# orottier/web-audio-api-rs

Measured on AMD Instinct MI355X. Metric: render quanta/sec (48kHz, 128-frame), higher is better.
Workload: dtype f64

## Files before the change

web-audio-api-rs_amd/csrc/waa_internal.hpp:

```cpp
#pragma once
#include <cstdint>
#include <cstdlib>

#include "waa_conv_noise.hpp"

namespace waa {

inline const char* measure_switch(const char* name) {
#ifdef WAA_MEASURE
  return getenv(name);
#else
  (void)name;
  return nullptr;
#endif
}

void raise_lds_limit(const void* kernel);

constexpr int RQ = 128;
constexpr int TILE_K = 32;
constexpr int TILE = 64 * TILE_K;
constexpr int QUANTA_PER_TILE = TILE / RQ;
constexpr int MAX_OPS = 12;
constexpr int MAX_INPUTS = 4;
// ... 29 lines not shown
struct SrcSchedule {
  const QRec* qrec;
  const SlowRec* slow;
  const uint8_t* tile_fast;
};
struct SrcInst {
  const float* base;
  uint64_t ch_stride;
  uint64_t frames;
  uint32_t sched;
  uint32_t aligned;
  SrcSchedule sc;
  int64_t linear_start;
  uint32_t fast_prefix;
  uint32_t linear_all;
};

enum : int32_t { IN_SILENT = 0, IN_SIGNAL = 1, IN_SOURCE = 2, IN_CONSTANT = 3, IN_DELAYED = 4 };
struct InputRef {
  int32_t kind;
  int32_t nch;
  SignalRef sig;
  const SrcInst* src;
  const SrcSchedule* sched;
  ParamRef offset;
  const int64_t* active;
  double sample_rate;
  int32_t num_quanta;
  int32_t feedback;
  uint64_t valid;
  ParamRef gain;
  int32_t has_gain;
  uint32_t fast_tiles;
  float delay_lo, delay_hi;
};

enum : int32_t {
  OP_GAIN = 1,
  OP_BIQUAD = 2,
  OP_WAVESHAPER = 3,
  OP_STEREO_PAN = 4,
  OP_PANNER = 5,
  OP_MIX = 6,
  OP_IIR = 7,
  OP_PARAM_ADD = 8
};
struct OpDesc {
  int32_t kind;
  int32_t nch_in;
  int32_t nch_out;
  int32_t i1;
  int32_t i2;
  int32_t i0;
  ParamRef p0;
  ParamRef p1;
  ParamRef p2;
  ParamRef p3;
  ParamRef p4;
  const void* ptr0;
  void* ptr1;
  const void* ptr2;
  uint64_t u0;
};

struct ChainDesc {
  int32_t n_inputs;
  int32_t in_nch;
  int32_t in_interp;
  int32_t n_ops;
  InputRef in[MAX_INPUTS];
  OpDesc ops[MAX_OPS];
  SignalRef out;
  uint32_t n_inst;
  uint32_t n_tiles;
  uint32_t n_quanta;
  uint32_t xcd_remap;
  uint32_t tile0, tile1;
  int32_t lds_curve_op;
  int32_t tile_major;
  uint32_t persist_block;
  uint32_t pad;
};

struct BiquadStreamDesc {
  InputRef in;
  const double* coefs;
  uint64_t coef_stride;
  int32_t vary;
  int32_t pad0;
  double* state;
  const double* hp;
  ParamRef gain[2];
  int32_t n_gain;
  int32_t nch;
  SignalRef out;
  uint32_t n_inst;
  uint32_t n_tiles;
  uint32_t n_quanta;
  uint32_t dup_out;
  uint32_t tile0, tile1;
};
void launch_biquad_stream(const BiquadStreamDesc& d, void* stream);
constexpr int BIQUAD_SCAN_PW = 88;
struct BiquadScanCtl {
  uint32_t* counter;
  uint32_t counter_base[8];
  double* payload;
  const double* pw;
  uint32_t* error;
};
void launch_biquad_scan_powers(const double* coefs, uint64_t coef_stride, double* pw, uint32_t n_inst, void* stream);
void launch_biquad_scan(const BiquadStreamDesc& d, const BiquadScanCtl& ctl, uint32_t* issued, void* stream);

constexpr int BIQUAD_HT_WORDS = 2 * TILE + 8;
struct BiquadLanesDesc {
  InputRef in;
  const double* coefs;
  double* ht;
  double* z;
  double* sin;
  double* state;
  ParamRef gain[2];
  int32_t n_gain, nch;
  SignalRef out;
  uint32_t n_inst, n_tiles, n_quanta, tile0, tile1;
  uint32_t fast_tiles;
  uint32_t lt0, lt1;
  uint32_t debug, pad;
};
void launch_biquad_tile_digest(const BiquadLanesDesc& d, void* stream);
void launch_biquad_lanes(const BiquadLanesDesc& d, void* stream);

struct IirStreamDesc {
  InputRef in;
  const double* coef;
  const double* pow;
  double* state;
  int32_t ns;
  int32_t nch;
  SignalRef out;
  uint32_t n_inst;
  uint32_t n_tiles;
  uint32_t n_quanta;
  uint32_t exact;
  uint32_t tile0, tile1;
  uint32_t coef_stride, pow_stride;
};
int iir_padded_states(int n_states);
void launch_iir_stream(const IirStreamDesc& d, void* stream);

struct CompRow {
  float thr, lo, hi, half_knee;
  float knee_partial, ratio, makeup, pad;
  float a_tau, a_one, r_tau, r_one;
};
struct CompDesc {
  SignalRef in;
  uint64_t in_valid;
  SignalRef out;
  float* xl;
  const CompRow* rows;
  uint32_t row_inst_stride, row_q_stride;
  uint32_t n_inst, n_quanta;
  uint64_t frames;
  uint32_t delay_frames;
  int32_t nch;
};
void launch_compressor_level(const CompDesc& d, void* stream);
void launch_compressor_detector(const CompDesc& d, void* stream);
void launch_compressor_apply(const CompDesc& d, void* stream);

enum : int32_t { RT_CHANNEL = 0, RT_DOWN2 = 1, RT_DOWN4 = 2, RT_DOWN6 = 3 };
struct RouteTerm {
  const float* base;
  uint64_t inst_stride, ch_stride;
  int32_t mode;
  int32_t ch;
};
struct RouteDesc {
  SignalRef out;
  const RouteTerm* terms;
  const uint32_t* row_off;
  uint32_t n_inst, rows;
  uint64_t frames;
};
void launch_route(const RouteDesc& d, void* stream);

struct ConvTerm {
  int32_t in_ch, ir_ch, out_ch, pad;
};
struct Cplx {
  float re, im;
};
struct ConvDesc {
  SignalRef in, out;
  int32_t n_terms;
  int32_t cin, cout;
  int32_t n;
  int32_t block;
  int32_t parts;
  int32_t nb;
  int32_t fft3;
  ConvTerm terms[4];
  const Cplx* H;
  Cplx* X;
  Cplx* Y;
  const Cplx* tw;
  const float* ir;
  uint64_t ir_len;
  uint64_t frames;
  uint64_t in_valid;
  uint32_t n_inst, n_pairs;
  int32_t ir_nch, pad1;
  int32_t kb0, kb1;
  int32_t mac_grid_order, pad2;
  const double* pre_coefs;
  uint64_t pre_coef_stride;
  double* pre_state;
  uint64_t ir_inst_stride;
  int32_t per_inst, pad3;
};
struct AnalyserDesc {
  SignalRef sig;
  uint32_t n_inst;
  int32_t fft_size;
  uint64_t frames_written;
  float smoothing;
  float min_db, max_db;
  int32_t pad;
  const float* window;
  const Cplx* tw;
  const Cplx* tw_full;
  const float* prev;
  float* db_out;
  uint8_t* byte_out;
  float* time_out;
  const uint8_t* code;
  uint64_t code_stride;
};
void launch_analyser(const AnalyserDesc& d, void* stream);
struct AnalyserSeriesDesc {
  AnalyserDesc a;
  int32_t first, hop;
  int32_t pulls;
  int32_t run;
  int32_t stage_span;
  int32_t lin;
  uint64_t frames;
  float* db_out;
  uint8_t* byte_out;
  float* time_out;
  uint8_t* tbyte_out;
};
void analyser_series_shape(AnalyserSeriesDesc* d);
void launch_analyser_series_fft(const AnalyserSeriesDesc& d, void* stream);
void launch_analyser_series_smooth(const AnalyserSeriesDesc& d, void* stream);
void launch_analyser_series_bytes(const AnalyserSeriesDesc& d, void* stream);
void launch_analyser_series_time(const AnalyserSeriesDesc& d, void* stream);
constexpr int DIRECT_MAX_TAPS = 128;
void launch_conv_direct(const ConvDesc& d, void* stream);
void launch_conv_ir_spectra(const ConvDesc& d, void* stream);
void launch_conv_forward(const ConvDesc& d, void* stream);
void launch_conv_mac(const ConvDesc& d, void* stream);
void launch_conv_inverse(const ConvDesc& d, void* stream);
void launch_conv3_ir_spectra(const ConvDesc& d, void* stream);
void launch_conv3_forward(const ConvDesc& d, void* stream);
void launch_conv3_inverse(const ConvDesc& d, void* stream);
void launch_conv_inst_direct(const ConvDesc& d, void* stream);
void launch_conv_inst_mac(const ConvDesc& d, void* stream);

struct DelayDesc {
  SignalRef in, out;
  ParamRef delay;
  double sample_rate;
  uint64_t frames;
  int32_t num_quanta;
  int32_t nch;
  uint32_t n_inst;
  uint32_t n_quanta;
  uint32_t tile0, tile1;
  int32_t in_cycle;
  int32_t pad;
  double quantum_duration;
};
void launch_delay(const DelayDesc& d, void* stream);


struct OscDesc {
  ParamRef frequency, detune;
  const double* start;
  const double* stop;
  const float* table;
  int32_t table_len;
  int32_t type;
  SignalRef out;
  uint64_t frames;
  uint32_t n_inst;
  uint32_t n_quanta;
  double sample_rate;
  const struct OscQuantum* table_q;
  const uint32_t* tq_row;
  const int64_t* active;
  const double* start_ratio;
  double* seg_phase;
  ParamRef post_gain[2];
  int32_t n_post;
  int32_t post_dup;
  const struct OscQuantum* fm_q;
  const uint32_t* fm_row;
  const float* fm_table;
  int32_t fm_table_len, fm_type;
  ParamRef fm_gain;
  int32_t fm_has_gain;
  float fm_min, fm_max, fm_default;
  int32_t pa_on;
  float pa_min, pa_max, pa_default;
  ParamRef pa_intrinsic;
};
constexpr int OSC_SEGMENTS = 8;
struct OscQuantum {
  double phase;
  double incr;
  int16_t first, end;
  int32_t outside_nyquist;
};
void launch_osc(const OscDesc& d, void* stream);

enum : int32_t { LI_NODE = 0, LI_DELAY_W = 1, LI_DELAY_R = 2 };
constexpr int LOOP_MAX_ITEMS = 24;
struct LoopItem {
  int32_t kind;
  int32_t nch_in;
  int32_t nch_out;
  int32_t interp;
  int32_t n_in;
  int32_t in_item[MAX_INPUTS];
  int32_t in_nch[MAX_INPUTS];
  SignalRef in_sig[MAX_INPUTS];
  SignalRef out;
  OpDesc op;
  int32_t writer_item;
  int32_t in_cycle;
  int32_t num_quanta;
  int32_t pad;
};
struct LoopDesc {
  const LoopItem* items;
  int32_t n_items;
  uint32_t n_inst;
  uint32_t n_quanta;
  uint32_t no_scan;
  double sample_rate;
  double quantum_duration;
};
void launch_loop(const LoopDesc& d, void* stream);

constexpr int DYN_MAX_IN = 8;
constexpr int DYN_MAX_ITEMS = 48;
constexpr int DYN_STATE = 20;
constexpr uint32_t CODE_SILENT = 0x80u;
enum : int32_t { DI_NODE = 0, DI_DELAY_W = 1, DI_DELAY_R = 2 };
enum : int32_t {
  DK_PASS = 0,
  DK_GAIN = 1, DK_BIQUAD = 2, DK_IIR = 3, DK_WAVESHAPER = 4, DK_STEREO_PAN = 5, DK_PANNER = 6,
  DK_CONV_IN = 7
};
struct DynInput {
  int32_t item;
  int32_t nch;
  SignalRef sig;
  const uint8_t* code;
  const uint32_t* remap;
  uint64_t code_stride;
};
struct DynItem {
  int32_t kind;
  int32_t dk;
  int32_t cc, mode, interp;
  int32_t n_in;
  int32_t nch_pub;
  int32_t publish_upmix;
  int32_t compact_ch1;
  int32_t flags;
  int32_t writer_item;
  int32_t in_cycle;
  int32_t num_quanta;
  int32_t pad;
  DynInput in[DYN_MAX_IN];
  OpDesc op;
  ParamRef alt1, alt2;
  SignalRef out;
  uint8_t* out_code;
  uint32_t* aux32;
  uint64_t code_stride;
  SignalRef xline;
  const uint32_t* xaux32;
  int32_t* xstate;
  int32_t pmod_n;
  int32_t pmod_item[4];
  float pmod_min, pmod_max, pmod_def;
};
struct DynDesc {
  const DynItem* items;
  int32_t n_items;
  uint32_t n_inst;
  uint32_t n_quanta;
  uint32_t no_scan;
  int32_t cmax;
  int32_t n_stages;
  int32_t stage_begin[9];
  int32_t pad;
  double sample_rate;
  double quantum_duration;
  unsigned long long* cycles;
  uint32_t q0, q1;
  double* save_f;
  int32_t* save_i;
  uint32_t split_ok, q_split;
};
void launch_dyn(const DynDesc& d, void* stream);
inline int dyn_planes(int cmax) { return cmax > 16 ? 32 : cmax > 8 ? 16 : cmax > 6 ? 8 : cmax > 2 ? 6 : 2; }
constexpr int DYN_MAX_STAGES = 8;
size_t dyn_lds_bytes(int n_items, int cmax, int stages = 1);
struct ConvCodeDesc {
  const uint8_t* in_code;
  uint8_t* out_code;
  uint64_t code_stride;
  uint64_t impulse_length;
  int32_t ir_nch;
  uint32_t n_inst, n_quanta;
  int32_t cout;
  uint8_t* clean;
  SignalRef out;
  uint32_t q0, q1;
  int32_t* state;
  int32_t noise, in_test_nch;
  SignalRef in;
  ConvNoiseIr nir[4];
};
constexpr int CONV_CODE_STATE_INTS = 4 + 4 * 4;
void launch_conv_codes(const ConvCodeDesc& d, void* stream);

struct BiquadCoefDesc {
  ParamRef frequency, detune, q, gain;
  double* coefs;
  uint64_t n_frames;
  uint64_t frames_padded;
  uint32_t rows;
  int32_t type;
  float sample_rate;
  int32_t lane_major;
};
void launch_biquad_coefs(const BiquadCoefDesc& d, void* stream);
constexpr int HP_WORDS = 72;
struct BiquadHpDesc {
  const double* coefs;
  double* hp;
  uint32_t n_tiles;
  uint32_t pad;
};
void launch_biquad_hp(const BiquadHpDesc& d, void* stream);

struct PannerGeomDesc {
  ParamRef p[15];
  const uint8_t* single;
  uint64_t single_stride;
  const uint8_t* dev_len[9];
  float *az, *gl_mono, *gr_mono, *gl_stereo, *gr_stereo, *dg, *cg;
  uint64_t n_frames;
  uint32_t rows;
  int32_t distance_model;
  double ref_distance, max_distance, rolloff;
  float cone_inner, cone_outer, cone_outer_gain;
  int32_t pad;
};
void launch_panner_geom(const PannerGeomDesc& d, void* stream);

struct TlEvent {
  int32_t type;
  float value;
  double time;
  double time_constant;
  double cancel_time;
  double duration;
  int32_t cancelled;
  int32_t curve_off;
  int32_t curve_len;
  int32_t pad;
};
struct TlHeader {
  float minv, maxv, defv, intrinsic;
  int32_t a_rate;
  int32_t ev_off;
  int32_t n_events;
  int32_t pad;
};
struct TimelineDesc {
  const TlHeader* hdr;
  const TlEvent* events;
  TlEvent* work;
  const float* curves;
  float* out;
  uint8_t* lens;
  uint64_t out_stride;
  uint32_t rows;
  uint32_t n_quanta;
  double sample_rate;
};
void launch_timeline(const TimelineDesc& d, void* stream);

constexpr int32_t LINK_SKIP = -2, LINK_FRESH = -1;
struct LinkDesc {
  const uint8_t* in_code;
  uint8_t* out_code;
  int32_t* prev;
  uint64_t code_stride, prev_stride;
  uint32_t n_inst, n_quanta;
  int32_t kind;
  int32_t can_propagate_silence;
  uint32_t tail_frames;
  int32_t pad;
  uint32_t q0, q1;
  int32_t* state;
};
void launch_link(const LinkDesc& d, void* stream);

struct QGemmDesc {
  const float* A;
  const uint16_t* A16;
  int32_t M, Kh;
  const float* src;
  uint64_t src_inst, src_ch, src_q;
  float* dst;
  uint64_t dst_inst, dst_ch, dst_q;
  const int32_t* prev;
  uint64_t prev_stride;
  const float* curve;
  int32_t curve_n;
  int32_t nch;
  uint32_t n_inst, n_quanta;
};
void launch_qgemm(const QGemmDesc& d, void* stream);

struct OsFftDesc {
  const float* src;
  uint64_t src_inst, src_ch;
  float* dst;
  uint64_t dst_inst, dst_ch;
  const int32_t* prev;
  uint64_t prev_stride;
  const float* curve;
  int32_t curve_n;
  int32_t R;
  const float* tables;
  const float* tw256;
  float* trash;
  int32_t nch;
  uint32_t n_inst, n_quanta;
  uint32_t seg_len, n_seg;
  uint32_t q0, q1;
};
void launch_osfft(const OsFftDesc& d, void* stream);
size_t osfft_lds_bytes(int R, int curve_n);

struct HrtfQ {
  int32_t v[3];
  float w[3];
  float gain;
  int32_t pad;
};
constexpr int HRTF_MAX_TAPS = 1280;
struct HrtfDesc {
  SignalRef in, out;
  const uint8_t* in_code;
  uint64_t code_stride;
  const int32_t* prev;
  uint64_t prev_stride;
  const float* hrir;
  const float* hstatic;
  const HrtfQ* table;
  uint32_t rows, per_row;
  int32_t taps;
  uint32_t n_inst, n_quanta;
  uint32_t q0, q1;
  int32_t pad;
  const float* fft_tables;
  const float* tw256;
  float* trash;
  uint32_t seg_len, n_seg;
  uint32_t n_seg_pad, pad2;
  const int32_t* jmax;
};
void launch_hrtf(const HrtfDesc& d, void* stream);
void launch_hrtf_fft(const HrtfDesc& d, void* stream);
void launch_hrtf_fft_tables(const float* pairs, uint32_t pair_stride, int taps, uint32_t rows, const double* cs_sn, float* out, void* stream);

struct DecodeDesc {
  const int16_t* pcm;
  float* out;
  uint64_t frames;
  uint64_t target_frames;
  uint64_t out_item_stride, out_ch_stride;
  uint32_t nch, n_items;
  int32_t resample;
  float scale;
};
void launch_pcm16_resample(const DecodeDesc& d, void* stream);
struct EncodeDesc {
  const float* in;
  int16_t* pcm;
  uint64_t frames, in_item_stride, in_ch_stride;
  uint32_t nch_in, nch_out, n_items, pad;
};
void launch_pcm16_pack(const EncodeDesc& d, void* stream);

void launch_chain(const ChainDesc& d, int cmax, void* stream);
struct EchoTail {
  int32_t n_inputs, in_nch, in_interp, store_line;
  int32_t ring_frames, sub_frames;
  InputRef in[MAX_INPUTS];
  int32_t alias[MAX_INPUTS];
  SignalRef out;
// ... 96 lines not shown
```

web-audio-api-rs_amd/csrc/waa_osc.hip:

```cpp
#include <hip/hip_runtime.h>

#include "waa_internal.hpp"

namespace waa {

namespace {
__device__ __forceinline__ double unroll_phase(double phase) {
  if (phase >= 1.) return phase - 1.;
  if (phase < 0.) return phase + 1.;
  return phase;
}
__device__ __forceinline__ double unroll_phase_unbounded(double phase) {
  const double r = fmod(phase, 1.);
  return r < 0. ? r + 1. : r;
}
__device__ __forceinline__ double poly_blep(double t, double dt) {
  if (t < dt) {
    t /= dt;
    return t + t - t * t - 1.0;
  } else if (t > 1.0 - dt) {
    t = (t - 1.0) / dt;
    return __builtin_fma(t, t, t) + t + 1.0;
  }
  return 0.0;
}
__device__ __forceinline__ float table_sample(const float* table, int len, double phase) {
  const double position = phase * (double)len;
  const double floored = floor(position);
  const int prev_index = (int)floored >= len ? 0 : (int)floored;
  int next_index = prev_index + 1;
  if (next_index == len) next_index = 0;
  const float k = (float)(position - floored);
  return __builtin_fmaf(table[prev_index], 1.f - k, table[next_index] * k);
}
__device__ __forceinline__ float waveform_sample(int type, const float* table, int table_len, double phase, double phase_incr) {
  switch (type) {
    case 1: {
      double sample = phase < 0.5 ? 1.0 : -1.0;
      sample += poly_blep(phase, phase_incr);
      sample -= poly_blep(unroll_phase(phase + 0.5), phase_incr);
      return (float)sample;
    }
    case 2: {
      const double ph = unroll_phase(phase + 0.5);
      double sample = 2.0 * ph - 1.0;
      sample -= poly_blep(ph, phase_incr);
      return (float)sample;
    }
    case 3: {
      double sample = -4. * phase + 2.;
      if (sample > 1.)
        sample = 2. - sample;
      else if (sample < -1.)
        sample = -2. - sample;
      return (float)sample;
    }
    default: return table_sample(table, table_len, phase);
  }
}
__device__ __forceinline__ float waveform_sample(const OscDesc& d, double phase, double phase_incr) {
  return waveform_sample(d.type, d.table, d.table_len, phase, phase_incr);
}
}

namespace {
__device__ __forceinline__ void osc_store(const OscDesc& d, uint32_t inst, float* out, uint64_t f0, float (&r)[4]) {
#pragma unroll
  for (int k = 0; k < 2; k++)
    if (k < d.n_post) {
      const float g = d.post_gain[k].base[inst];
      const bool mute = fabsf(g) <= 1e-6f, pass = fabsf(1.f - g) <= 1e-6f;
#pragma unroll
      for (int e = 0; e < 4; e++) r[e] = mute ? 0.f : (pass ? r[e] : r[e] * g);
    }
  if (d.pa_on) {
    const uint32_t q = (uint32_t)(f0 / RQ), qc = q < d.n_quanta ? q : d.n_quanta - 1;
    const float iv = d.pa_intrinsic.mode == 0 ? d.pa_intrinsic.base[inst] : d.pa_intrinsic.base[(uint64_t)inst * d.pa_intrinsic.stride + qc];
#pragma unroll
    for (int e = 0; e < 4; e++) {
      const float o1 = r[e] + iv;
      r[e] = o1 != o1 ? d.pa_default : fminf(fmaxf(o1, d.pa_min), d.pa_max);
    }
  }
  *reinterpret_cast<float4*>(out + f0) = make_float4(r[0], r[1], r[2], r[3]);
  if (d.post_dup) *reinterpret_cast<float4*>(out + d.out.ch_stride + f0) = make_float4(r[0], r[1], r[2], r[3]);
}
}

__global__ __launch_bounds__(64) void osc_kernel(const OscDesc d) {
  const uint32_t inst = blockIdx.x * 64 + threadIdx.x;
  if (inst >= d.n_inst) return;
  __builtin_amdgcn_s_setreg(1 | (6 << 6) | (1 << 11), 0);
  float* out = d.out.base + (uint64_t)inst * d.out.inst_stride;
  double start_time = d.start[inst];
  const double stop_time = d.stop[inst];
  const double sample_rate = d.sample_rate, dt = 1. / sample_rate, nyquist = sample_rate / 2.;
  double phase = 0.;
  bool started = false;
  const bool per_frame = d.frequency.mode == 2 || d.detune.mode == 2;
  for (uint32_t q = 0; q < d.n_quanta; q++) {
    const uint64_t f0 = (uint64_t)q * RQ;
    const double block_time = (double)f0 / sample_rate;
    const double next_block_time = block_time + dt * (double)RQ;
    float4* o4 = reinterpret_cast<float4*>(out + f0);
    if (stop_time <= block_time || start_time >= next_block_time) {
      for (int j = 0; j < RQ / 4; j++) o4[j] = make_float4(0.f, 0.f, 0.f, 0.f);
      continue;
    }
    double current_time = block_time;
    if (!started && start_time < current_time) start_time = current_time;
    auto generate = [&](bool outside_nyquist, double phase_incr) __attribute__((always_inline)) -> float {
      float v = 0.f;
      if (!(current_time < start_time || current_time >= stop_time)) {
        if (!started) {
          if (current_time > start_time) {
            const double ratio = (current_time - start_time) / dt;
            phase = outside_nyquist ? unroll_phase_unbounded(phase_incr * ratio) : unroll_phase(phase_incr * ratio);
          }
          started = true;
        }
        v = outside_nyquist ? 0.f : waveform_sample(d, phase, phase_incr);
        phase = outside_nyquist ? unroll_phase_unbounded(phase + phase_incr) : unroll_phase(phase + phase_incr);
      }
      current_time += dt;
      return v;
    };
    if (!per_frame) {
      const float freq = d.frequency.mode == 0 ? d.frequency.base[inst] : d.frequency.base[(uint64_t)inst * d.frequency.stride + q];
      const float detune = d.detune.mode == 0 ? d.detune.base[inst] : d.detune.base[(uint64_t)inst * d.detune.stride + q];
      const double computed_freq = (double)freq * exp2((double)detune / 1200.);
      const double phase_incr = computed_freq / sample_rate;
      const bool outside_nyquist = fabs(computed_freq) >= nyquist;
      const bool fully_active = started && start_time <= block_time && stop_time >= next_block_time;
      if (fully_active && !outside_nyquist) {
        for (int j = 0; j < RQ / 4; j++) {
          float r[4];
#pragma unroll
          for (int e = 0; e < 4; e++) {
            r[e] = waveform_sample(d, phase, phase_incr);
            phase = unroll_phase(phase + phase_incr);
          }
          o4[j] = make_float4(r[0], r[1], r[2], r[3]);
        }
      } else {
        for (int j = 0; j < RQ / 4; j++) {
          float r[4];
#pragma unroll
          for (int e = 0; e < 4; e++) r[e] = generate(outside_nyquist, phase_incr);
          o4[j] = make_float4(r[0], r[1], r[2], r[3]);
        }
      }
    } else {
      for (int j = 0; j < RQ / 4; j++) {
        float r[4];
#pragma unroll
        for (int e = 0; e < 4; e++) {
          const uint64_t f = f0 + j * 4 + e;
          const float freq = d.frequency.mode == 0   ? d.frequency.base[inst]
                             : d.frequency.mode == 1 ? d.frequency.base[(uint64_t)inst * d.frequency.stride + q]
                                                     : d.frequency.base[(uint64_t)inst * d.frequency.stride + f];
          const float detune = d.detune.mode == 0   ? d.detune.base[inst]
                               : d.detune.mode == 1 ? d.detune.base[(uint64_t)inst * d.detune.stride + q]
                                                    : d.detune.base[(uint64_t)inst * d.detune.stride + f];
          const double computed_freq = (double)freq * exp2((double)detune / 1200.);
          const double phase_incr = computed_freq / sample_rate;
          r[e] = generate(fabs(computed_freq) >= nyquist, phase_incr);
        }
        o4[j] = make_float4(r[0], r[1], r[2], r[3]);
      }
    }
  }
  for (uint64_t f = (uint64_t)d.n_quanta * RQ; f < d.frames; f += 4) *reinterpret_cast<float4*>(out + f) = make_float4(0.f, 0.f, 0.f, 0.f);
}

__global__ __launch_bounds__(256) void osc_par_kernel(const OscDesc d) {
  const uint32_t inst = blockIdx.y;
  const uint64_t f0 = ((uint64_t)blockIdx.x * 256 + threadIdx.x) * 4;
  if (f0 >= d.frames) return;
  __builtin_amdgcn_s_setreg(1 | (6 << 6) | (1 << 11), 0);
  float* out = d.out.base + (uint64_t)inst * d.out.inst_stride;
  const uint32_t q = (uint32_t)(f0 / RQ);
  float r[4] = {0.f, 0.f, 0.f, 0.f};
  if (q < d.n_quanta) {
    const OscQuantum oq = d.table_q[(uint64_t)d.tq_row[inst] * d.n_quanta + q];
    const int i0 = (int)(f0 % RQ);
#pragma unroll
    for (int e = 0; e < 4; e++) {
      const int i = i0 + e;
      if (i >= oq.first && i < oq.end && !oq.outside_nyquist) {
        const double x = __builtin_fma((double)(i - oq.first), oq.incr, oq.phase);
        double ph = x - floor(x);
        if (ph >= 1.) ph -= 1.;
        r[e] = waveform_sample(d, ph, oq.incr);
      }
    }
  }
  osc_store(d, inst, out, f0, r);
}

template <int PASS>
__global__ __launch_bounds__(64) void osc_scan_kernel(const OscDesc d) {
  const uint32_t inst = blockIdx.x;
  const uint32_t seg = blockIdx.y;
  const int lane = threadIdx.x;
  __builtin_amdgcn_s_setreg(1 | (6 << 6) | (1 << 11), 0);
  float* out = d.out.base + (uint64_t)inst * d.out.inst_stride;
  const int64_t first = d.active[(uint64_t)inst * 2], end = d.active[(uint64_t)inst * 2 + 1];
  const double ratio = d.start_ratio[inst];
  const double sample_rate = d.sample_rate, nyquist = sample_rate / 2.;
  const uint64_t groups = (d.frames + 255) / 256, per_seg = (groups + OSC_SEGMENTS - 1) / OSC_SEGMENTS;
  const uint64_t g_begin = (uint64_t)seg * per_seg * 256, g_end = g_begin + per_seg * 256 < d.frames ? g_begin + per_seg * 256 : d.frames;
  double carry = 0.;
  if (PASS == 1) {
    for (uint32_t sgm = 0; sgm < seg; sgm++) {
      carry += d.seg_phase[(uint64_t)inst * OSC_SEGMENTS + sgm];
      carry -= floor(carry);
    }
  }
  const bool det_const = d.detune.mode == 0;
  const double det_mul = det_const ? exp2((double)d.detune.base[inst] / 1200.) : 1.;
  for (uint64_t g0 = g_begin; g0 < g_end; g0 += 256) {
    const uint64_t f0 = g0 + (uint64_t)lane * 4;
    double incr[4];
    bool outside[4];
    OscQuantum mq4{};
    if (d.fm_q) {
      const uint64_t fq = f0 < (uint64_t)d.n_quanta * RQ ? f0 : (uint64_t)d.n_quanta * RQ - 1;
      mq4 = d.fm_q[(uint64_t)d.fm_row[inst] * d.n_quanta + fq / RQ];
    }
#pragma unroll
    for (int e = 0; e < 4; e++) {
      const uint64_t f = f0 + e;
      const uint64_t fc = f < (uint64_t)d.n_quanta * RQ ? f : (uint64_t)d.n_quanta * RQ - 1;
      const uint32_t q = (uint32_t)(fc / RQ);
      float freq = d.frequency.mode == 0   ? d.frequency.base[inst]
                   : d.frequency.mode == 1 ? d.frequency.base[(uint64_t)inst * d.frequency.stride + q]
                                           : d.frequency.base[(uint64_t)inst * d.frequency.stride + fc];
      if (d.fm_q) {
        const OscQuantum& mq = mq4;
        const int i = (int)(fc % RQ);
        float m = 0.f;
        if (i >= mq.first && i < mq.end && !mq.outside_nyquist) {
          const double x = __builtin_fma((double)(i - mq.first), mq.incr, mq.phase);
          double ph = x - floor(x);
          if (ph >= 1.) ph -= 1.;
          m = waveform_sample(d.fm_type, d.fm_table, d.fm_table_len, ph, mq.incr);
        }
        if (d.fm_has_gain) {
          const float g = d.fm_gain.mode == 0 ? d.fm_gain.base[inst] : d.fm_gain.base[(uint64_t)inst * d.fm_gain.stride + q];
          m = fabsf(g) <= 1e-6f ? 0.f : (fabsf(1.f - g) <= 1e-6f ? m : m * g);
        }
        float o1 = m + freq;
        freq = o1 != o1 ? d.fm_default : fminf(fmaxf(o1, d.fm_min), d.fm_max);
      }
      double computed_freq;
      if (det_const) {
        computed_freq = (double)freq * det_mul;
      } else {
        const float detune = d.detune.mode == 1 ? d.detune.base[(uint64_t)inst * d.detune.stride + q]
                                                : d.detune.base[(uint64_t)inst * d.detune.stride + fc];
        computed_freq = (double)freq * exp2((double)detune / 1200.);
      }
      incr[e] = computed_freq / sample_rate;
      outside[e] = fabs(computed_freq) >= nyquist;
    }
    double adv[4];
#pragma unroll
    for (int e = 0; e < 4; e++) {
      const int64_t f = (int64_t)(f0 + e);
      adv[e] = (f >= first && f < end) ? incr[e] : 0.;
      if (f == first) adv[e] += incr[e] * ratio;
    }
    const double local = ((adv[0] + adv[1]) + adv[2]) + adv[3];
    double incl = local;
#pragma unroll
    for (int sft = 1; sft < 64; sft <<= 1) {
      const double t = __shfl_up(incl, sft, 64);
      if (lane >= sft) incl += t;
    }
    if (PASS == 1) {
      double ph = carry + (incl - local);
      float r[4];
#pragma unroll
      for (int e = 0; e < 4; e++) {
        const int64_t f = (int64_t)(f0 + e);
        double p = ph;
        if (f == first) p += incr[e] * ratio;
        p -= floor(p);
        if (p >= 1.) p -= 1.;
        r[e] = (f >= first && f < end && !outside[e]) ? waveform_sample(d, p, incr[e]) : 0.f;
        ph += adv[e];
      }
      osc_store(d, inst, out, f0, r);
    }
    double total = __shfl(incl, 63, 64) + carry;
    total -= floor(total);
    carry = total;
  }
  if (PASS == 0 && lane == 0) d.seg_phase[(uint64_t)inst * OSC_SEGMENTS + seg] = carry;
}

void launch_osc(const OscDesc& d, void* stream) {
  if (d.table_q) {
    hipLaunchKernelGGL(osc_par_kernel, dim3((unsigned)((d.frames + 1023) / 1024), d.n_inst), dim3(256), 0, (hipStream_t)stream, d);
    return;
  }
  if (d.active) {
    hipLaunchKernelGGL(osc_scan_kernel<0>, dim3(d.n_inst, OSC_SEGMENTS), dim3(64), 0, (hipStream_t)stream, d);
    hipLaunchKernelGGL(osc_scan_kernel<1>, dim3(d.n_inst, OSC_SEGMENTS), dim3(64), 0, (hipStream_t)stream, d);
    return;
  }
  hipLaunchKernelGGL(osc_kernel, dim3((d.n_inst + 63) / 64), dim3(64), 0, (hipStream_t)stream, d);
}

}
```

web-audio-api-rs_amd/csrc/waa_plan_sources.cpp:

```cpp
#include <array>
#include <set>

#include "waa_host.hpp"
#include "waa_plan_parts.hpp"

namespace waa {
namespace host {

int widen_narrow_buffers(waa_batch* b, Node& n, uint32_t nch) {
  std::map<const float*, DeviceBuffer> done;
  for (auto& bf : n.bufs) {
    if (!bf.valid || bf.nch >= nch) continue;
    auto it = done.find(bf.base);
    if (it == done.end()) {
      const uint64_t stride = std::max<uint64_t>(bf.ch_stride, 4);
      float* d = nullptr;
      int e = dev_alloc(b, &d, (size_t)nch * stride, true);
      if (e) return e;
      const size_t all = (size_t)nch * stride * sizeof(float), plane = (size_t)bf.frames * sizeof(float);
      if (b->dry) {
        std::memset(d, 0, all);
        for (uint32_t c = 0; c < bf.nch && plane; c++) std::memcpy(d + (size_t)c * stride, bf.base + (size_t)c * bf.ch_stride, plane);
      } else {
        HIP_TRY(hipMemsetAsync(d, 0, all, b->stream));
// ... 130 lines not shown
      linear_all.push_back(all ? 1u : 0u);
      plan_note(b, "source node %u schedule %zu: tiles [0, %u) are one linear run from buffer frame %lld%s", id, scheds.size(), prefix,
                (long long)start0, all && prefix < b->n_tiles ? " (and so is the rest of the render)" : "");
    }
    SrcSchedule ds{};
    QRec* dq = nullptr;
    int e = dev_upload(b, &dq, so.qrec);
    if (e) return e;
    ds.qrec = dq;
    if (so.any_slow) {
      SlowRec* dsr = nullptr;
      e = dev_upload(b, &dsr, so.slow);
      if (e) return e;
      ds.slow = dsr;
    }
    uint8_t* dtf = nullptr;
    e = dev_upload(b, &dtf, so.tile_fast);
    if (e) return e;
    ds.tile_fast = dtf;
    si.sched = (uint32_t)scheds.size();
    scheds.push_back(ds);
    if (!automated) {
      dedup[key] = si.sched;
      last_key = key;
      last_sched = si.sched;
      last_key_valid = true;
    }
  }
  for (auto& si : insts) {
    si.sc = scheds[si.sched];
    si.linear_start = linear[si.sched].first;
    si.fast_prefix = si.aligned && !measure_switch("WAA_NO_LINEAR_PREFIX") ? linear[si.sched].second : 0;
    si.linear_all = si.fast_prefix ? linear_all[si.sched] : 0;
  }
  SrcInst* d_insts = nullptr;
  int e = dev_upload(b, &d_insts, insts);
  if (e) return e;
  SrcSchedule* d_scheds = nullptr;
  e = dev_upload(b, &d_scheds, scheds);
  if (e) return e;
  in->src = d_insts;
  in->sched = d_scheds;
  b->src_tables[d_insts] = insts;
#ifdef WAA_MEASURE
  b->src_table_of_node[id] = d_insts;
#endif
  in->fast_tiles = b->n_tiles;
  for (auto& si : insts) in->fast_tiles = std::min(in->fast_tiles, !si.base ? 0u : (si.linear_all ? b->n_tiles : si.fast_prefix));
  plan_note(b, "source node %u: %zu distinct schedule(s) for %u instance(s)", id, scheds.size(), b->n_inst);
  return 0;
}

int reduce_fan_in(waa_batch* b, std::vector<InputRef>& ins, int in_nch, int interp) {
  while (ins.size() > (size_t)MAX_INPUTS) {
    float* ptr = nullptr;
    int e = dev_alloc(b, &ptr, (size_t)b->n_inst * in_nch * b->lp);
    if (e) return e;
    const SignalRef part{ptr, (uint64_t)in_nch * b->lp, b->lp, in_nch, 0};
    if ((e = push_chain_step(b, std::vector<InputRef>(ins.begin(), ins.begin() + MAX_INPUTS), in_nch, interp, {}, part))) return e;
    InputRef partial{};
    partial.kind = IN_SIGNAL;
    partial.nch = in_nch;
    partial.sig = part;
    ins.erase(ins.begin(), ins.begin() + MAX_INPUTS);
    ins.insert(ins.begin(), partial);
    plan_note(b, "fan-in partial sum of %d inputs -> %dch", MAX_INPUTS, in_nch);
  }
  return 0;
}

int node_input_signal(waa_batch* b, uint32_t id, SignalRef* out_sig, const SignalRef* target, uint64_t* valid) {
  Node& n = b->nodes[id];
  if (valid) *valid = b->lp;
  if (!target && n.in_edges.size() == 1) {
    Node& p = b->nodes[b->edges[n.in_edges[0]].from];
    if (p.is_view && valid) {
      *out_sig = p.view_sig;
      *valid = p.view_valid;
      return 0;
    }
    if (p.materialized && p.out_nch == n.in_nch) {
      *out_sig = p.sig;
      return 0;
    }
  }
  SignalRef in_sig;
  int e = 0;
  if (target)
    in_sig = *target;
  else
    e = temp_signal(b, n.in_nch, &in_sig);
  if (e) return e;
  std::vector<InputRef> ins;
  if (n.in_edges.empty()) {
    InputRef in{};
    in.kind = IN_SILENT;
    in.nch = 1;
    ins.push_back(in);
  } else {
    for (int ie : n.in_edges) {
      InputRef in{};
      if ((e = build_edge_input(b, id, ie, &in))) return e;
      ins.push_back(in);
    }
    if ((e = premix_ordered_inputs(b, id, ins))) return e;
    if ((e = reduce_fan_in(b, ins, n.in_nch, n.interp))) return e;
  }
  if ((e = push_chain_step(b, ins, n.in_nch, n.interp, {}, in_sig))) return e;
  *out_sig = in_sig;
  return 0;
}

static inline bool osc_quantum_fully_active(double block_time, double next_block_time, double start_time, double stop_time, double dt) {
  return start_time <= block_time && stop_time >= next_block_time + dt;
}

int plan_oscillator(waa_batch* b, uint32_t id) {
  const bool check_replay = measure_switch("WAA_OSC_PLAN_CHECK") != nullptr;
  Node& n = b->nodes[id];
  Step st;
  st.kind = StepKind::Osc;
  OscDesc& d = st.osc;
  std::memset(&d, 0, sizeof d);
  int e;
  if ((e = node_param(b, id, WAA_PARAM_OSCILLATOR_FREQUENCY, &d.frequency)) ||
      (e = node_param(b, id, WAA_PARAM_OSCILLATOR_DETUNE, &d.detune)))
    return e;
  std::vector<double> start(b->n_inst), stop(b->n_inst);
  for (uint32_t i = 0; i < b->n_inst; i++) {
    start[i] = n.sched[i].start;
    stop[i] = n.sched[i].stop;
  }
  double *d_start = nullptr, *d_stop = nullptr;
  if ((e = dev_upload(b, &d_start, start)) || (e = dev_upload(b, &d_stop, stop))) return e;
  d.start = d_start;
  d.stop = d_stop;
  d.type = n.osc_wave.empty() ? n.desc.i[0] : WAA_OSC_CUSTOM;
  if (d.type == WAA_OSC_CUSTOM && n.osc_wave.empty())
    return fail(WAA_ERR_INVALID_STATE, "InvalidStateError - custom oscillator %u has no PeriodicWave", id);
  std::vector<float> table;
  if (d.type == WAA_OSC_CUSTOM) {
    table = n.osc_wave;
  } else {
    table.resize(2048);
    const float pi = 3.14159265358979323846f;
    for (int x = 0; x < 2048; x++) table[x] = std::sin(((float)x) * 2.0f * pi * (1.f / 2048.f));
  }
  float* d_table = nullptr;
  if ((e = dev_upload(b, &d_table, table))) return e;
  d.table = d_table;
  d.table_len = (int32_t)table.size();
  d.out = n.sig;
  d.frames = b->lp;
  d.n_inst = b->n_inst;
  d.n_quanta = b->n_quanta;
  d.sample_rate = (double)b->sr;
  const bool parallel = d.frequency.mode != 2 && d.detune.mode != 2 && !getenv("WAA_OSC_EXACT");
  if (parallel) {
    std::vector<OscQuantum> tq;
    std::vector<uint32_t> row_of(b->n_inst, 0);
    const double sample_rate = (double)b->sr, dt = 1. / sample_rate, nyquist = sample_rate / 2.;
    auto frac = [](long double x) {
      long double r = x - floorl(x);
      return (double)(r >= 1.L ? r - 1.L : r);
    };
    std::map<std::array<double, 4>, uint32_t> replayed;
    for (uint32_t i = 0; i < b->n_inst; i++) {
      const auto fq = param_per_quantum(b, n.params[WAA_PARAM_OSCILLATOR_FREQUENCY], i, nullptr);
      const auto dq = param_per_quantum(b, n.params[WAA_PARAM_OSCILLATOR_DETUNE], i, nullptr);
      double start_time = start[i];
      const double stop_time = stop[i];
      if (fq.size() == 1 && dq.size() == 1) {
        const std::array<double, 4> key = {start_time, stop_time, (double)fq[0], (double)dq[0]};
        auto it = replayed.find(key);
        if (it != replayed.end()) {
          row_of[i] = it->second;
          continue;
        }
        replayed.emplace(key, (uint32_t)(tq.size() / b->n_quanta));
      }
      const size_t row = tq.size() / b->n_quanta;
      row_of[i] = (uint32_t)row;
      tq.resize(tq.size() + b->n_quanta);
      long double phase = 0.L;
      bool started = false;
      for (uint32_t q = 0; q < b->n_quanta; q++) {
        OscQuantum& oq = tq[row * b->n_quanta + q];
        oq = OscQuantum{0., 0., 0, 0, 0};
        const double block_time = (double)((uint64_t)q * RQ) / sample_rate;
        const double next_block_time = block_time + dt * (double)RQ;
        if (stop_time <= block_time || start_time >= next_block_time) continue;
        if (!started && start_time < block_time) start_time = block_time;
        const float f = fq[fq.size() == 1 ? 0 : q], det = dq[dq.size() == 1 ? 0 : q];
        const double computed_freq = (double)f * std::exp2((double)det / 1200.);
        const double incr = computed_freq / sample_rate;
        oq.incr = incr;
        oq.outside_nyquist = std::fabs(computed_freq) >= nyquist ? 1 : 0;
        int first = -1, end = RQ;
        if (osc_quantum_fully_active(block_time, next_block_time, start_time, stop_time, dt) && !check_replay) {
          first = 0;
          started = true;
        } else {
          const bool expect_full = osc_quantum_fully_active(block_time, next_block_time, start_time, stop_time, dt);
          const bool was_started = started;
          double current_time = block_time;
          for (int k = 0; k < RQ; k++) {
            const bool active = !(current_time < start_time || current_time >= stop_time);
            if (active && first < 0) {
              first = k;
              if (!started) {
                if (current_time > start_time) {
                  if (expect_full) return fail(WAA_ERR_INVALID_STATE, "internal: oscillator replay shortcut (sub-sample start)");
                  phase = frac((long double)incr * (long double)((current_time - start_time) / dt));
                }
                started = true;
              }
            }
            if (!active && first >= 0) {
              end = k;
              break;
            }
            current_time += dt;
          }
          (void)was_started;
          if (expect_full && !(first == 0 && end == RQ)) return fail(WAA_ERR_INVALID_STATE, "internal: oscillator replay shortcut (range)");
        }
        if (first < 0) continue;
        oq.first = (int16_t)first;
        oq.end = (int16_t)end;
        oq.phase = (double)phase;
        phase = frac(phase + (long double)(end - first) * (long double)incr);
      }
    }
    OscQuantum* d_tq = nullptr;
    uint32_t* d_row = nullptr;
    if ((e = dev_upload(b, &d_tq, tq)) || (e = dev_upload(b, &d_row, row_of))) return e;
    d.table_q = d_tq;
    d.tq_row = d_row;
  }
  const bool scan = !parallel && !getenv("WAA_OSC_EXACT");
  if (scan) {
    std::vector<int64_t> act((size_t)b->n_inst * 2, 0);
    std::vector<double> ratio(b->n_inst, 0.);
    const double sample_rate = (double)b->sr, dt = 1. / sample_rate;
    std::map<std::pair<double, double>, uint32_t> clock_of;
    for (uint32_t i = 0; i < b->n_inst; i++) {
      double start_time = start[i];
      const double stop_time = stop[i];
      {
        auto it = clock_of.find({start_time, stop_time});
        if (it != clock_of.end()) {
          act[(size_t)i * 2] = act[(size_t)it->second * 2];
          act[(size_t)i * 2 + 1] = act[(size_t)it->second * 2 + 1];
          ratio[i] = ratio[it->second];
          continue;
        }
        clock_of.emplace(std::make_pair(start_time, stop_time), i);
      }
      int64_t first = -1, end = -1;
      bool started = false;
      for (uint32_t q = 0; q < b->n_quanta; q++) {
        const double block_time = (double)((uint64_t)q * RQ) / sample_rate;
        const double next_block_time = block_time + dt * (double)RQ;
        if (stop_time <= block_time || start_time >= next_block_time) continue;
        if (!started && start_time < block_time) start_time = block_time;
        if (osc_quantum_fully_active(block_time, next_block_time, start_time, stop_time, dt) && !check_replay) {
          if (first < 0) {
            first = (int64_t)q * RQ;
            started = true;
          }
          end = (int64_t)(q + 1) * RQ;
          continue;
        }
        const bool expect_full = osc_quantum_fully_active(block_time, next_block_time, start_time, stop_time, dt);
        const int64_t end_before = end;
        double current_time = block_time;
        for (int k = 0; k < RQ; k++) {
          const bool active = !(current_time < start_time || current_time >= stop_time);
          if (active) {
            if (first < 0) {
              first = (int64_t)q * RQ + k;
              if (current_time > start_time) {
                if (expect_full) return fail(WAA_ERR_INVALID_STATE, "internal: oscillator replay shortcut (sub-sample start)");
                ratio[i] = (current_time - start_time) / dt;
              }
              started = true;
            }
            end = (int64_t)q * RQ + k + 1;
          }
          current_time += dt;
        }
        (void)end_before;
        if (expect_full && !(end == (int64_t)(q + 1) * RQ && first <= (int64_t)q * RQ))
          return fail(WAA_ERR_INVALID_STATE, "internal: oscillator replay shortcut (range)");
      }
      act[(size_t)i * 2] = first < 0 ? 0 : first;
      act[(size_t)i * 2 + 1] = first < 0 ? 0 : end;
    }
    int64_t* d_act = nullptr;
    double* d_ratio = nullptr;
    if ((e = dev_upload(b, &d_act, act)) || (e = dev_upload(b, &d_ratio, ratio))) return e;
    d.active = d_act;
    d.start_ratio = d_ratio;
    double* d_seg = nullptr;
    if ((e = dev_alloc(b, &d_seg, (size_t)b->n_inst * OSC_SEGMENTS))) return e;
    d.seg_phase = d_seg;
  }
  st.profile_slot = slot_for(b, parallel ? "osc_par_kernel" : scan ? "osc_scan_kernel" : "osc_kernel");
  n.osc_step = (parallel || scan) ? (int)b->steps.size() : -1;
  b->steps.push_back(st);
  static const char* names[] = {"sine", "square", "sawtooth", "triangle", "custom"};
  plan_note(b, "oscillator node %u: %s (%s) frequency=%s detune=%s", id, names[d.type],
            parallel ? "time-parallel, closed-form phase" : scan ? "prefix-sum phase" : "lane per instance, serial phase",
            d.frequency.mode == 0 ? "const" : d.frequency.mode == 1 ? "k-rate" : "a-rate",
            d.detune.mode == 0 ? "const" : d.detune.mode == 1 ? "k-rate" : "a-rate");
  return 0;
}

void fuse_fm_operators(waa_batch* b) {
  if (measure_switch("WAA_NO_FM_FOLD")) return;
  for (size_t c = 0; c < b->steps.size(); c++) {
    Step& cs = b->steps[c];
    if (cs.kind != StepKind::Osc || !cs.osc.active || cs.osc.frequency.mode != 2 || cs.osc.fm_q || cs.group >= 0) continue;
    const void* table = cs.osc.frequency.base;
    int pi = -1, mi = -1;
    for (size_t k = 0; k < c; k++) {
      const Step& st = b->steps[k];
      if (st.kind == StepKind::Chain && st.group < 0 && !st.echo_fused && (const void*)st.chain.out.base == table) pi = (int)k;
    }
    if (pi < 0) continue;
    Step& ps = b->steps[(size_t)pi];
    const ChainDesc& ch = ps.chain;
    if (ch.n_ops != 1 || ch.ops[0].kind != OP_PARAM_ADD || ch.n_inputs != 1 || ch.in_nch != 1 || ch.in[0].kind != IN_SIGNAL ||
        ch.in[0].nch != 1 || ch.out.inst_stride != cs.osc.frequency.stride || ch.ops[0].p0.mode > 1 ||
        (ch.in[0].has_gain && ch.in[0].gain.mode > 1) || (ch.in[0].valid != 0 && ch.in[0].valid < (uint64_t)b->n_quanta * RQ))
      continue;
    for (size_t k = 0; k < (size_t)pi; k++) {
      const Step& st = b->steps[k];
      if (st.kind == StepKind::Osc && st.group < 0 && !st.echo_fused && st.osc.table_q && st.osc.out.base == ch.in[0].sig.base) mi = (int)k;
    }
    if (mi < 0) continue;
    Step& ms = b->steps[(size_t)mi];
    if (ms.osc.n_post != 0 || ms.osc.post_dup || ms.osc.out.nch != 1 || ms.osc.out.inst_stride != ch.in[0].sig.inst_stride) continue;
    bool shared = false;
    for (size_t k = 0; k < b->steps.size() && !shared; k++) {
      if ((int)k == pi || k == c) continue;
      const StepIo io = step_io(b, b->steps[k]);
      for (const void* r : io.reads) shared |= r == table || ((int)k != pi && r == (const void*)ms.osc.out.base);
    }
    {
      const StepIo io = step_io(b, cs);
      for (const void* r : io.reads) shared |= r == (const void*)ms.osc.out.base;
    }
    for (const Node& an : b->nodes)
      if (an.live && (an.desc.kind == WAA_NODE_ANALYSER || an.desc.kind == WAA_NODE_DESTINATION) &&
          (an.sig.base == ms.osc.out.base || (const void*)an.sig.base == table))
        shared = true;
    if (shared) continue;
    OscDesc& d = cs.osc;
    d.fm_q = ms.osc.table_q;
    d.fm_row = ms.osc.tq_row;
    d.fm_table = ms.osc.table;
    d.fm_table_len = ms.osc.table_len;
    d.fm_type = ms.osc.type;
    d.fm_has_gain = ch.in[0].has_gain ? 1 : 0;
    d.fm_gain = ch.in[0].gain;
    std::memcpy(&d.fm_min, &ch.ops[0].i0, 4);
    std::memcpy(&d.fm_max, &ch.ops[0].i1, 4);
    std::memcpy(&d.fm_default, &ch.ops[0].i2, 4);
    d.frequency = ch.ops[0].p0;
    ms.echo_fused = true;
    ps.echo_fused = true;
    plan_note(b, "FM: launches %d (the modulating oscillator) and %d (the frequency param's sum) are folded into the carrier's prefix-sum kernel (launch %zu): modulator, %sparam sum and clamp per frame in registers",
              mi, pi, c, d.fm_has_gain ? "edge gain, " : "");
  }
}

void fuse_lfo_params(waa_batch* b) {
  if (measure_switch("WAA_NO_LFO_FOLD")) return;
  for (size_t pi = 0; pi < b->steps.size(); pi++) {
    Step& ps = b->steps[pi];
    if (ps.kind != StepKind::Chain || ps.group >= 0 || ps.echo_fused) continue;
    const ChainDesc& ch = ps.chain;
    if (ch.n_ops != 1 || ch.ops[0].kind != OP_PARAM_ADD || ch.n_inputs != 1 || ch.in_nch != 1 || ch.in[0].kind != IN_SIGNAL ||
        ch.in[0].nch != 1 || ch.out.nch != 1 || ch.ops[0].p0.mode > 1 || (ch.in[0].has_gain && ch.in[0].gain.mode != 0) ||
        (ch.in[0].valid != 0 && ch.in[0].valid < (uint64_t)b->n_quanta * RQ))
      continue;
    int mi = -1;
    for (size_t k = 0; k < pi; k++) {
      const Step& st = b->steps[k];
      if (st.kind == StepKind::Osc && st.group < 0 && !st.echo_fused && st.osc.table_q && !st.osc.pa_on && st.osc.out.base == ch.in[0].sig.base) mi = (int)k;
    }
    if (mi < 0) continue;
    Step& ms = b->steps[(size_t)mi];
    if (ms.osc.post_dup || ms.osc.out.nch != 1 || ms.osc.n_post + (ch.in[0].has_gain ? 1 : 0) > 2 ||
        ms.osc.out.inst_stride != ch.in[0].sig.inst_stride || ch.out.inst_stride != ms.osc.out.inst_stride)
      continue;
    bool shared = false;
    for (size_t k = 0; k < b->steps.size() && !shared; k++) {
      if (k == pi) continue;
      const StepIo io = step_io(b, b->steps[k]);
      for (const void* r : io.reads) shared |= r == (const void*)ms.osc.out.base;
    }
    for (const Node& an : b->nodes)
      if (an.live && (an.desc.kind == WAA_NODE_ANALYSER || an.desc.kind == WAA_NODE_DESTINATION) && an.sig.base == ms.osc.out.base) shared = true;
    if (shared) continue;
    OscDesc& d = ms.osc;
    if (ch.in[0].has_gain) d.post_gain[d.n_post++] = ch.in[0].gain;
    d.pa_on = 1;
    d.pa_intrinsic = ch.ops[0].p0;
    std::memcpy(&d.pa_min, &ch.ops[0].i0, 4);
    std::memcpy(&d.pa_max, &ch.ops[0].i1, 4);
    std::memcpy(&d.pa_default, &ch.ops[0].i2, 4);
    d.out = ch.out;
    ps.echo_fused = true;
    plan_note(b, "LFO: launch %zu (the param's sum: %sintrinsic value, clamp) is folded into the store of the oscillator that drives it (launch %d)", pi,
              ch.in[0].has_gain ? "depth gain, " : "", mi);
  }
}

}
}
```

Baseline: 2.895 billion.

## Replace two-pass segmented oscillator phase scan with single-pass block-wide tiled scan

Replaces the two launches of the segmented prefix-sum oscillator kernel with one kernel per instance that uses 8 waves. Each wave computes increments and a lane scan for several 256-frame groups and keeps them in registers. The waves then exchange tile totals through shared memory behind a barrier, and each wave renders with its carried phase. This removes one kernel launch, the recomputation of increments in the second pass, and the global seg_phase round trip. In exchange it adds per-tile barriers, register pressure from the kept groups, and only one block per instance, which limits parallelism when there are few instances.

```diff
diff --git a/web-audio-api-rs_amd/csrc/waa_internal.hpp b/web-audio-api-rs_amd/csrc/waa_internal.hpp
--- a/web-audio-api-rs_amd/csrc/waa_internal.hpp
+++ b/web-audio-api-rs_amd/csrc/waa_internal.hpp
@@ -355,7 +355,9 @@
   const uint32_t* tq_row;
   const int64_t* active;
   const double* start_ratio;
+#ifdef WAA_MEASURE
   double* seg_phase;
+#endif
   ParamRef post_gain[2];
   int32_t n_post;
   int32_t post_dup;
@@ -370,7 +372,12 @@
   float pa_min, pa_max, pa_default;
   ParamRef pa_intrinsic;
 };
+constexpr int OSC_WAVES = 8;
+constexpr int OSC_GROUPS = 4;
+constexpr int OSC_TILE = OSC_WAVES * OSC_GROUPS * 256;
+#ifdef WAA_MEASURE
 constexpr int OSC_SEGMENTS = 8;
+#endif
 struct OscQuantum {
   double phase;
   double incr;
diff --git a/web-audio-api-rs_amd/csrc/waa_osc.hip b/web-audio-api-rs_amd/csrc/waa_osc.hip
--- a/web-audio-api-rs_amd/csrc/waa_osc.hip
+++ b/web-audio-api-rs_amd/csrc/waa_osc.hip
@@ -198,6 +198,167 @@
   osc_store(d, inst, out, f0, r);
 }
 
+namespace {
+__device__ __forceinline__ void osc_increments(const OscDesc& d, uint32_t inst, uint64_t f0, bool det_const, double det_mul, double sample_rate,
+                                               double nyquist, double (&incr)[4], bool (&outside)[4]) {
+  OscQuantum mq4{};
+  if (d.fm_q) {
+    const uint64_t fq = f0 < (uint64_t)d.n_quanta * RQ ? f0 : (uint64_t)d.n_quanta * RQ - 1;
+    mq4 = d.fm_q[(uint64_t)d.fm_row[inst] * d.n_quanta + fq / RQ];
+  }
+#pragma unroll
+  for (int e = 0; e < 4; e++) {
+    const uint64_t f = f0 + e;
+    const uint64_t fc = f < (uint64_t)d.n_quanta * RQ ? f : (uint64_t)d.n_quanta * RQ - 1;
+    const uint32_t q = (uint32_t)(fc / RQ);
+    float freq = d.frequency.mode == 0   ? d.frequency.base[inst]
+                 : d.frequency.mode == 1 ? d.frequency.base[(uint64_t)inst * d.frequency.stride + q]
+                                         : d.frequency.base[(uint64_t)inst * d.frequency.stride + fc];
+    if (d.fm_q) {
+      const OscQuantum& mq = mq4;
+      const int i = (int)(fc % RQ);
+      float m = 0.f;
+      if (i >= mq.first && i < mq.end && !mq.outside_nyquist) {
+        const double x = __builtin_fma((double)(i - mq.first), mq.incr, mq.phase);
+        double ph = x - floor(x);
+        if (ph >= 1.) ph -= 1.;
+        m = waveform_sample(d.fm_type, d.fm_table, d.fm_table_len, ph, mq.incr);
+      }
+      if (d.fm_has_gain) {
+        const float g = d.fm_gain.mode == 0 ? d.fm_gain.base[inst] : d.fm_gain.base[(uint64_t)inst * d.fm_gain.stride + q];
+        m = fabsf(g) <= 1e-6f ? 0.f : (fabsf(1.f - g) <= 1e-6f ? m : m * g);
+      }
+      float o1 = m + freq;
+      freq = o1 != o1 ? d.fm_default : fminf(fmaxf(o1, d.fm_min), d.fm_max);
+    }
+    double computed_freq;
+    if (det_const) {
+      computed_freq = (double)freq * det_mul;
+    } else {
+      const float detune = d.detune.mode == 1 ? d.detune.base[(uint64_t)inst * d.detune.stride + q]
+                                              : d.detune.base[(uint64_t)inst * d.detune.stride + fc];
+      computed_freq = (double)freq * exp2((double)detune / 1200.);
+    }
+    incr[e] = computed_freq / sample_rate;
+    outside[e] = fabs(computed_freq) >= nyquist;
+  }
+}
+__device__ __forceinline__ void osc_advances(uint64_t f0, int64_t first, int64_t end, double ratio, const double (&incr)[4], double (&adv)[4]) {
+#pragma unroll
+  for (int e = 0; e < 4; e++) {
+    const int64_t f = (int64_t)(f0 + e);
+    adv[e] = (f >= first && f < end) ? incr[e] : 0.;
+    if (f == first) adv[e] += incr[e] * ratio;
+  }
+}
+__device__ __forceinline__ double osc_lane_scan(double local, int lane) {
+  double incl = local;
+#pragma unroll
+  for (int sft = 1; sft < 64; sft <<= 1) {
+    const double t = __shfl_up(incl, sft, 64);
+    if (lane >= sft) incl += t;
+  }
+  return incl;
+}
+__device__ __forceinline__ void osc_render4(const OscDesc& d, uint32_t inst, float* out, uint64_t f0, int64_t first, int64_t end, double ratio,
+                                            double ph, const double (&incr)[4], const bool (&outside)[4], const double (&adv)[4]) {
+  float r[4];
+#pragma unroll
+  for (int e = 0; e < 4; e++) {
+    const int64_t f = (int64_t)(f0 + e);
+    double p = ph;
+    if (f == first) p += incr[e] * ratio;
+    p -= floor(p);
+    if (p >= 1.) p -= 1.;
+    r[e] = (f >= first && f < end && !outside[e]) ? waveform_sample(d, p, incr[e]) : 0.f;
+    ph += adv[e];
+  }
+  osc_store(d, inst, out, f0, r);
+}
+__device__ __forceinline__ void osc_barrier() { asm volatile("s_waitcnt lgkmcnt(0)\n\ts_barrier" ::: "memory"); }
+}
+
+__global__ __launch_bounds__(OSC_WAVES * 64) __attribute__((amdgpu_waves_per_eu(4, 4))) void osc_one_pass_kernel(const OscDesc d) {
+  static_assert(OSC_TILE == 8192, "tests/test_oscillator_one_pass.py mirrors the tile length");
+  static_assert(OSC_GROUPS >= 1 && OSC_GROUPS <= 8, "the Nyquist flags of a tile's groups are 4 bits each of one register");
+  __shared__ double tile_adv[2][OSC_WAVES];
+  struct Group {
+    double incr[4];
+    double excl;
+  };
+  const uint32_t inst = blockIdx.x;
+  const int lane = threadIdx.x & 63;
+  const int wave = __builtin_amdgcn_readfirstlane(threadIdx.x >> 6);
+  __builtin_amdgcn_s_setreg(1 | (6 << 6) | (1 << 11), 0);
+  float* out = d.out.base + (uint64_t)inst * d.out.inst_stride;
+  const int64_t first = d.active[(uint64_t)inst * 2], end = d.active[(uint64_t)inst * 2 + 1];
+  const double ratio = d.start_ratio[inst];
+  const double sample_rate = d.sample_rate, nyquist = sample_rate / 2.;
+  const bool det_const = d.detune.mode == 0;
+  const double det_mul = det_const ? exp2((double)d.detune.base[inst] / 1200.) : 1.;
+  const uint64_t n_tiles = (d.frames + OSC_TILE - 1) / OSC_TILE;
+  Group kept[OSC_GROUPS] = {};
+  uint32_t flags = 0;
+  double carry = 0.;
+  for (uint64_t t = 0; t < n_tiles; t++) {
+    const uint64_t w0 = t * OSC_TILE + (uint64_t)wave * (OSC_GROUPS * 256);
+    double advance = 0.;
+#pragma unroll 1
+    for (int k = 0; k < OSC_GROUPS; k++) {
+      const uint64_t g0 = w0 + (uint64_t)k * 256;
+      Group cur = {};
+      uint32_t bits = 0;
+      if (g0 < d.frames) {
+        const uint64_t f0 = g0 + (uint64_t)lane * 4;
+        bool outside[4];
+        osc_increments(d, inst, f0, det_const, det_mul, sample_rate, nyquist, cur.incr, outside);
+        double adv[4];
+        osc_advances(f0, first, end, ratio, cur.incr, adv);
+        const double local = ((adv[0] + adv[1]) + adv[2]) + adv[3];
+        const double incl = osc_lane_scan(local, lane);
+        cur.excl = advance + (incl - local);
+        double total = __shfl(incl, 63, 64) + advance;
+        total -= floor(total);
+        advance = total;
+#pragma unroll
+        for (int e = 0; e < 4; e++) bits |= outside[e] ? 1u << e : 0u;
+      }
+#pragma unroll
+      for (int j = OSC_GROUPS - 1; j > 0; j--) kept[j] = kept[j - 1];
+      kept[0] = cur;
+      flags = flags << 4 | bits;
+    }
+    if (lane == 0) tile_adv[t & 1][wave] = advance;
+    osc_barrier();
+    double mine = carry;
+#pragma unroll
+    for (int w = 0; w < OSC_WAVES; w++) {
+      if (w == wave) mine = carry;
+      carry += tile_adv[t & 1][w];
+      carry -= floor(carry);
+    }
+#pragma unroll 1
+    for (int k = 0; k < OSC_GROUPS; k++) {
+      const uint64_t g0 = w0 + (uint64_t)k * 256;
+      const Group cur = kept[OSC_GROUPS - 1];
+      const uint32_t bits = flags >> 4 * (OSC_GROUPS - 1) & 15u;
+#pragma unroll
+      for (int j = OSC_GROUPS - 1; j > 0; j--) kept[j] = kept[j - 1];
+      flags <<= 4;
+      if (g0 < d.frames) {
+        const uint64_t f0 = g0 + (uint64_t)lane * 4;
+        bool outside[4];
+#pragma unroll
+        for (int e = 0; e < 4; e++) outside[e] = (bits >> e & 1u) != 0;
+        double adv[4];
+        osc_advances(f0, first, end, ratio, cur.incr, adv);
+        if (f0 < d.frames) osc_render4(d, inst, out, f0, first, end, ratio, mine + cur.excl, cur.incr, outside, adv);
+      }
+    }
+  }
+}
+
+#ifdef WAA_MEASURE
 template <int PASS>
 __global__ __launch_bounds__(64) void osc_scan_kernel(const OscDesc d) {
   const uint32_t inst = blockIdx.x;
@@ -223,82 +384,19 @@
     const uint64_t f0 = g0 + (uint64_t)lane * 4;
     double incr[4];
     bool outside[4];
-    OscQuantum mq4{};
-    if (d.fm_q) {
-      const uint64_t fq = f0 < (uint64_t)d.n_quanta * RQ ? f0 : (uint64_t)d.n_quanta * RQ - 1;
-      mq4 = d.fm_q[(uint64_t)d.fm_row[inst] * d.n_quanta + fq / RQ];
-    }
-#pragma unroll
-    for (int e = 0; e < 4; e++) {
-      const uint64_t f = f0 + e;
-      const uint64_t fc = f < (uint64_t)d.n_quanta * RQ ? f : (uint64_t)d.n_quanta * RQ - 1;
-      const uint32_t q = (uint32_t)(fc / RQ);
-      float freq = d.frequency.mode == 0   ? d.frequency.base[inst]
-                   : d.frequency.mode == 1 ? d.frequency.base[(uint64_t)inst * d.frequency.stride + q]
-                                           : d.frequency.base[(uint64_t)inst * d.frequency.stride + fc];
-      if (d.fm_q) {
-        const OscQuantum& mq = mq4;
-        const int i = (int)(fc % RQ);
-        float m = 0.f;
-        if (i >= mq.first && i < mq.end && !mq.outside_nyquist) {
-          const double x = __builtin_fma((double)(i - mq.first), mq.incr, mq.phase);
-          double ph = x - floor(x);
-          if (ph >= 1.) ph -= 1.;
-          m = waveform_sample(d.fm_type, d.fm_table, d.fm_table_len, ph, mq.incr);
-        }
-        if (d.fm_has_gain) {
-          const float g = d.fm_gain.mode == 0 ? d.fm_gain.base[inst] : d.fm_gain.base[(uint64_t)inst * d.fm_gain.stride + q];
-          m = fabsf(g) <= 1e-6f ? 0.f : (fabsf(1.f - g) <= 1e-6f ? m : m * g);
-        }
-        float o1 = m + freq;
-        freq = o1 != o1 ? d.fm_default : fminf(fmaxf(o1, d.fm_min), d.fm_max);
-      }
-      double computed_freq;
-      if (det_const) {
-        computed_freq = (double)freq * det_mul;
-      } else {
-        const float detune = d.detune.mode == 1 ? d.detune.base[(uint64_t)inst * d.detune.stride + q]
-                                                : d.detune.base[(uint64_t)inst * d.detune.stride + fc];
-        computed_freq = (double)freq * exp2((double)detune / 1200.);
-      }
-      incr[e] = computed_freq / sample_rate;
-      outside[e] = fabs(computed_freq) >= nyquist;
-    }
+    osc_increments(d, inst, f0, det_const, det_mul, sample_rate, nyquist, incr, outside);
     double adv[4];
-#pragma unroll
-    for (int e = 0; e < 4; e++) {
-      const int64_t f = (int64_t)(f0 + e);
-      adv[e] = (f >= first && f < end) ? incr[e] : 0.;
-      if (f == first) adv[e] += incr[e] * ratio;
-    }
+    osc_advances(f0, first, end, ratio, incr, adv);
     const double local = ((adv[0] + adv[1]) + adv[2]) + adv[3];
-    double incl = local;
-#pragma unroll
-    for (int sft = 1; sft < 64; sft <<= 1) {
-      const double t = __shfl_up(incl, sft, 64);
-      if (lane >= sft) incl += t;
-    }
-    if (PASS == 1) {
-      double ph = carry + (incl - local);
-      float r[4];
-#pragma unroll
-      for (int e = 0; e < 4; e++) {
-        const int64_t f = (int64_t)(f0 + e);
-        double p = ph;
-        if (f == first) p += incr[e] * ratio;
-        p -= floor(p);
-        if (p >= 1.) p -= 1.;
-        r[e] = (f >= first && f < end && !outside[e]) ? waveform_sample(d, p, incr[e]) : 0.f;
-        ph += adv[e];
-      }
-      osc_store(d, inst, out, f0, r);
-    }
+    const double incl = osc_lane_scan(local, lane);
+    if (PASS == 1) osc_render4(d, inst, out, f0, first, end, ratio, carry + (incl - local), incr, outside, adv);
     double total = __shfl(incl, 63, 64) + carry;
     total -= floor(total);
     carry = total;
   }
   if (PASS == 0 && lane == 0) d.seg_phase[(uint64_t)inst * OSC_SEGMENTS + seg] = carry;
 }
+#endif
 
 void launch_osc(const OscDesc& d, void* stream) {
   if (d.table_q) {
@@ -306,8 +404,14 @@
     return;
   }
   if (d.active) {
-    hipLaunchKernelGGL(osc_scan_kernel<0>, dim3(d.n_inst, OSC_SEGMENTS), dim3(64), 0, (hipStream_t)stream, d);
-    hipLaunchKernelGGL(osc_scan_kernel<1>, dim3(d.n_inst, OSC_SEGMENTS), dim3(64), 0, (hipStream_t)stream, d);
+#ifdef WAA_MEASURE
+    if (d.seg_phase) {
+      hipLaunchKernelGGL(osc_scan_kernel<0>, dim3(d.n_inst, OSC_SEGMENTS), dim3(64), 0, (hipStream_t)stream, d);
+      hipLaunchKernelGGL(osc_scan_kernel<1>, dim3(d.n_inst, OSC_SEGMENTS), dim3(64), 0, (hipStream_t)stream, d);
+      return;
+    }
+#endif
+    hipLaunchKernelGGL(osc_one_pass_kernel, dim3(d.n_inst), dim3(OSC_WAVES * 64), 0, (hipStream_t)stream, d);
     return;
   }
   hipLaunchKernelGGL(osc_kernel, dim3((d.n_inst + 63) / 64), dim3(64), 0, (hipStream_t)stream, d);
diff --git a/web-audio-api-rs_amd/csrc/waa_plan_sources.cpp b/web-audio-api-rs_amd/csrc/waa_plan_sources.cpp
--- a/web-audio-api-rs_amd/csrc/waa_plan_sources.cpp
+++ b/web-audio-api-rs_amd/csrc/waa_plan_sources.cpp
@@ -456,9 +456,13 @@
     if ((e = dev_upload(b, &d_act, act)) || (e = dev_upload(b, &d_ratio, ratio))) return e;
     d.active = d_act;
     d.start_ratio = d_ratio;
-    double* d_seg = nullptr;
-    if ((e = dev_alloc(b, &d_seg, (size_t)b->n_inst * OSC_SEGMENTS))) return e;
-    d.seg_phase = d_seg;
+#ifdef WAA_MEASURE
+    if (measure_switch("WAA_OSC_TWO_PASS")) {
+      double* d_seg = nullptr;
+      if ((e = dev_alloc(b, &d_seg, (size_t)b->n_inst * OSC_SEGMENTS))) return e;
+      d.seg_phase = d_seg;
+    }
+#endif
   }
   st.profile_slot = slot_for(b, parallel ? "osc_par_kernel" : scan ? "osc_scan_kernel" : "osc_kernel");
   n.osc_step = (parallel || scan) ? (int)b->steps.size() : -1;
@@ -468,6 +472,9 @@
             parallel ? "time-parallel, closed-form phase" : scan ? "prefix-sum phase" : "lane per instance, serial phase",
             d.frequency.mode == 0 ? "const" : d.frequency.mode == 1 ? "k-rate" : "a-rate",
             d.detune.mode == 0 ? "const" : d.detune.mode == 1 ? "k-rate" : "a-rate");
+#ifdef WAA_MEASURE
+  if (d.seg_phase) plan_note(b, "oscillator node %u: two-pass segment form (WAA_OSC_TWO_PASS)", id);
+#endif
   return 0;
 }
 
```

Result: no change. 2.900 billion (median of 2 runs) (+0.2%).
